# RajaeeKh/TriNerfLet

Measured on NVIDIA B200. Metric: rays/sec per training step (fwd+bwd), higher is better.
Workload: dtype f16

## Files before the change

### trinerflet_b200/csrc/idwt.cu

```cuda
#include "common.cuh"
#include "idwt_core.cuh"
#include <stdlib.h>

#include <type_traits>

namespace tnl {

template <typename Cfg, int W>
__global__ void __launch_bounds__(Cfg::NT, (768 / Cfg::NT) > 0 ? (768 / Cfg::NT) : 1)
k_idwt_fwd(const float* __restrict__ x, const float* __restrict__ yh, float* __restrict__ out, int n, int C,
           int rows_per_cta, float* __restrict__ abs_sum, const int4* __restrict__ items, const int* __restrict__ n_items) {
    extern __shared__ __align__(16) float smem[];
    float* mid0 = smem;
    float* stage0 = smem + 2 * Cfg::MID_F;
    const int tid = threadIdx.x;
    IdwtGeom g;
    if (items != nullptr) {
        const int chunks = C / Cfg::CG;
        const int idx = blockIdx.x / chunks;
        if (idx >= __ldg(n_items)) return;
        const int4 it = __ldg(items + idx);
        g = idwt_geom_item<Cfg>(tid, blockIdx.x % chunks, IdwtItem{it.x, it.y, it.z, it.w}, n, C);
    } else {
        g = idwt_geom<Cfg>(tid, IdwtBlock{(int)blockIdx.x, (int)blockIdx.y, (int)blockIdx.z}, n, C, rows_per_cta);
    }
    FwdState st;
    fwd_state_init<Cfg>(st, g, x, yh, tid);
    fwd_issue_stage<Cfg>(g, st, stage0, tid);
    fwd_issue_stage<Cfg>(g, st, stage0 + Cfg::STAGE, tid);
    for (int s = 0; s < g.nsteps; s += 3) {
#define TNL_STEP(PH)                                                                          \
    if (s + PH < g.nsteps) {                                                                  \
        const int ss = s + PH;                                                                \
        fwd_issue_stage<Cfg>(g, st, stage0 + ((PH + 2) % 3) * Cfg::STAGE, tid);               \
        cp_async_wait<2>();                                                                   \
        float* mid = mid0 + (ss & 1) * Cfg::MID_F;                                            \
        fwd_phase_a<Cfg, PH, W>(g, st, stage0 + PH * Cfg::STAGE, mid, tid, ss);               \
        __syncthreads();                                                                      \
        fwd_phase_b<Cfg, W>(g, st, mid, out, ss);                                             \
    }
        TNL_STEP(0) TNL_STEP(1) TNL_STEP(2)
#undef TNL_STEP
    }
    cp_async_wait<0>();
    if (abs_sum != nullptr) {
        float v = st.abs_acc;
#pragma unroll
        for (int o = 16; o > 0; o >>= 1) v += __shfl_xor_sync(0xffffffffu, v, o);
        __syncthreads();
        if ((tid & 31) == 0) smem[tid >> 5] = v;
        __syncthreads();
        if (tid < 32) {
            float w = tid < (Cfg::NT + 31) / 32 ? smem[tid] : 0.f;
#pragma unroll
            for (int o = 16; o > 0; o >>= 1) w += __shfl_xor_sync(0xffffffffu, w, o);
            if (tid == 0) atomicAdd(abs_sum, w);
        }
    }
}

template <typename Cfg, int W>
__global__ void __launch_bounds__(Cfg::NT, (768 / Cfg::NT) > 0 ? (768 / Cfg::NT) : 1)
k_idwt_bwd(const float* __restrict__ gout, float* __restrict__ g_x, float* __restrict__ g_yh, int n, int C,
           int rows_per_cta, const float* __restrict__ yh, const float* __restrict__ reg_grad, float reg_coef, int plane0,
           const int4* __restrict__ items, const int* __restrict__ n_items) {
    extern __shared__ __align__(16) float smem[];
    float* mid0 = smem;
    float* stage0 = smem + 2 * Cfg::MID_B;
    const int tid = threadIdx.x;
    IdwtGeom g;
    if (items != nullptr) {
        const int chunks = C / Cfg::CG;
        const int idx = blockIdx.x / chunks;
        if (idx >= __ldg(n_items)) return;
        const int4 it = __ldg(items + idx);
        g = idwt_geom_item<Cfg>(tid, blockIdx.x % chunks, IdwtItem{it.x, it.y, it.z, it.w}, n, C);
    } else {
        g = idwt_geom<Cfg>(tid, IdwtBlock{(int)blockIdx.x, (int)blockIdx.y, (int)blockIdx.z + plane0}, n, C, rows_per_cta);
    }
    BwdState st;
    bwd_state_init<Cfg>(st, g, gout);
    const float reg = (yh != nullptr && reg_grad != nullptr) ? reg_coef * __ldg(reg_grad) : 0.f;
    const float* yh_reg = (yh != nullptr && reg_grad != nullptr) ? yh : nullptr;
    bwd_issue_stage<Cfg>(g, st, stage0, tid);
    bwd_issue_stage<Cfg>(g, st, stage0 + Cfg::STAGE, tid);
    for (int s = 0; s < g.nsteps; s += 3) {
#define TNL_STEP(PH)                                                                          \
    if (s + PH < g.nsteps) {                                                                  \
        const int ss = s + PH;                                                                \
        bwd_issue_stage<Cfg>(g, st, stage0 + ((PH + 2) % 3) * Cfg::STAGE, tid);               \
        cp_async_wait<2>();                                                                   \
        float* mid = mid0 + (ss & 1) * Cfg::MID_B;                                            \
        bwd_phase_a<Cfg, PH, W>(st, stage0 + PH * Cfg::STAGE, mid, tid);                      \
        __syncthreads();                                                                      \
        bwd_phase_b<Cfg, W>(g, mid, g_x, g_yh, tid, ss, yh_reg, reg);                         \
    }
        TNL_STEP(0) TNL_STEP(1) TNL_STEP(2)
#undef TNL_STEP
    }
    cp_async_wait<0>();
}

__global__ void __launch_bounds__(256)
k_idwt_clean_fwd(const float* __restrict__ yh, int n, int C, const int4* __restrict__ items, const int* __restrict__ n_items,
                 float* __restrict__ abs_sum) {
    __shared__ float red[8];
    const int cnt = __ldg(n_items);
    const int warp = threadIdx.x >> 5, lane = threadIdx.x & 31;
    float acc = 0.f;
    const int run4 = 16 * C / 4;
    for (int idx = blockIdx.x; idx < cnt; idx += gridDim.x) {
        const int4 it = __ldg(items + idx);
        const int rows = min(it.w, n) - it.z;
        for (int rb = warp; rb < 3 * rows; rb += 8) {
            const int b = rb / rows, r = rb - b * rows;
            const float4* src = reinterpret_cast<const float4*>(yh + (((size_t)(it.x * 3 + b) * n + it.z + r) * n + it.y) * C);
            for (int q = lane; q < run4; q += 32) {
                const float4 v = __ldg(src + q);
                acc += fabsf(v.x) + fabsf(v.y) + fabsf(v.z) + fabsf(v.w);
            }
        }
    }
#pragma unroll
    for (int o = 16; o > 0; o >>= 1) acc += __shfl_xor_sync(0xffffffffu, acc, o);
    if (lane == 0) red[warp] = acc;
    __syncthreads();
    if (threadIdx.x < 32) {
        float w = threadIdx.x < 8 ? red[threadIdx.x] : 0.f;
// ... 74 lines not shown
    cudaFuncSetAttribute(k_idwt_bwd<Cfg, W>, cudaFuncAttributeMaxDynamicSharedMemorySize, (int)Cfg::SMEM_B);
    if (max_active > 0 && (parts & 1u))
        k_idwt_bwd<Cfg, W><<<max_active * (C / Cfg::CG), Cfg::NT, Cfg::SMEM_B, stream>>>(g, g_x, g_yh, (int)n, (int)C, 0, yh, reg_grad, reg_coef,
                                                                                     0, reinterpret_cast<const int4*>(active), counts);
    if (max_clean > 0 && (parts & 2u))
        k_idwt_clean_bwd<<<min(max_clean, (uint32_t)kNumSM * 8u), 256, 0, stream>>>(yh, g_x, g_yh, (int)n, (int)C,
                                                                                   reinterpret_cast<const int4*>(clean), counts + 1, reg_grad,
                                                                                   reg_coef, abs_sum);
    return finish_launch("idwt_level_backward_sparse");
}

template <typename Cfg, int W>
static int launch_fwd(const float* x, const float* yh, float* out, uint32_t n, uint32_t C, float* abs_sum,
                      cudaStream_t stream) {
    cudaFuncSetAttribute(k_idwt_fwd<Cfg, W>, cudaFuncAttributeMaxDynamicSharedMemorySize, (int)Cfg::SMEM_F);
    unsigned gx, gy, gz, rows;
    idwt_grid<Cfg>(n, C, kNumSM, gx, gy, gz, rows);
    k_idwt_fwd<Cfg, W><<<dim3(gx, gy, gz), Cfg::NT, Cfg::SMEM_F, stream>>>(x, yh, out, (int)n, (int)C, (int)rows, abs_sum, nullptr, nullptr);
    return finish_launch("idwt_level_forward");
}

template <typename Cfg, int W>
static int launch_bwd(const float* g, float* g_x, float* g_yh, uint32_t n, uint32_t C, const float* yh,
                      const float* reg_grad, float reg_coef, uint32_t plane0, uint32_t nplanes, cudaStream_t stream) {
    cudaFuncSetAttribute(k_idwt_bwd<Cfg, W>, cudaFuncAttributeMaxDynamicSharedMemorySize, (int)Cfg::SMEM_B);
    unsigned gx, gy, gz, rows;
    idwt_grid<Cfg>(n, C, kNumSM, gx, gy, gz, rows);
    gz = nplanes;
    k_idwt_bwd<Cfg, W><<<dim3(gx, gy, gz), Cfg::NT, Cfg::SMEM_B, stream>>>(g, g_x, g_yh, (int)n, (int)C, (int)rows, yh, reg_grad,
                                                                        reg_coef, (int)plane0, nullptr, nullptr);
    return finish_launch("idwt_level_backward");
}

template <typename Fn>
static int with_wavelet(uint32_t wavelet, Fn&& fn) {
    switch (wavelet) {
        case TNL_WAVELET_BIOR6_8: return fn(std::integral_constant<int, TNL_WAVELET_BIOR6_8>());
        case TNL_WAVELET_HAAR: return fn(std::integral_constant<int, TNL_WAVELET_HAAR>());
        case TNL_WAVELET_BIOR2_2: return fn(std::integral_constant<int, TNL_WAVELET_BIOR2_2>());
        case TNL_WAVELET_BIOR2_6: return fn(std::integral_constant<int, TNL_WAVELET_BIOR2_6>());
        case TNL_WAVELET_BIOR4_4: return fn(std::integral_constant<int, TNL_WAVELET_BIOR4_4>());
        default: set_error("idwt: unknown wavelet id %u", wavelet); return TNL_ERR_INVALID_ARGUMENT;
    }
}

}

using namespace tnl;

extern "C" {

int tnl_idwt_level_forward_wavelet(const float* x, const float* yh, float* out, uint32_t n, uint32_t C, float* abs_sum,
                                   uint32_t wavelet, tnl_stream_t stream) {
    TNL_ARG_CHECK(x && yh && out, "null pointer");
    TNL_ARG_CHECK(n >= 8 && n % 8 == 0 && n <= 16384, "n must be a multiple of 8 in [8, 16384]");
    TNL_ARG_CHECK(C >= 8 && C % 8 == 0, "C must be a multiple of 8");
    cudaStream_t s = reinterpret_cast<cudaStream_t>(stream);
    return with_wavelet(wavelet, [&](auto w) {
        constexpr int W = decltype(w)::value;
        if (C % 32 == 0 && getenv("TNL_IDWT_CG32")) return launch_fwd<IdwtCfg<32, 32>, W>(x, yh, out, n, C, abs_sum, s);
        if (C % 24 == 0) return launch_fwd<IdwtCfg<24, 32>, W>(x, yh, out, n, C, abs_sum, s);
        if (C % 16 == 0) return launch_fwd<IdwtCfg<16, 32>, W>(x, yh, out, n, C, abs_sum, s);
        return launch_fwd<IdwtCfg<8, 32>, W>(x, yh, out, n, C, abs_sum, s);
    });
}

int tnl_idwt_level_backward_wavelet(const float* g_out, float* g_x, float* g_yh, uint32_t n, uint32_t C, const float* yh,
                                    const float* reg_grad, float reg_coef, uint32_t plane0, uint32_t nplanes, uint32_t wavelet,
                                    tnl_stream_t stream) {
    TNL_ARG_CHECK(nplanes >= 1 && plane0 + nplanes <= 3, "plane range must lie in [0, 3)");
    TNL_ARG_CHECK(g_out && g_x && g_yh, "null pointer");
    TNL_ARG_CHECK(n >= 8 && n % 8 == 0 && n <= 16384, "n must be a multiple of 8 in [8, 16384]");
    TNL_ARG_CHECK(C >= 8 && C % 8 == 0, "C must be a multiple of 8");
    cudaStream_t s = reinterpret_cast<cudaStream_t>(stream);
    return with_wavelet(wavelet, [&](auto w) {
        constexpr int W = decltype(w)::value;
        if (C % 32 == 0 && getenv("TNL_IDWT_CG32"))
            return launch_bwd<IdwtCfg<32, 32>, W>(g_out, g_x, g_yh, n, C, yh, reg_grad, reg_coef, plane0, nplanes, s);
        if (C % 24 == 0) return launch_bwd<IdwtCfg<24, 32>, W>(g_out, g_x, g_yh, n, C, yh, reg_grad, reg_coef, plane0, nplanes, s);
        if (C % 16 == 0) return launch_bwd<IdwtCfg<16, 32>, W>(g_out, g_x, g_yh, n, C, yh, reg_grad, reg_coef, plane0, nplanes, s);
        return launch_bwd<IdwtCfg<8, 32>, W>(g_out, g_x, g_yh, n, C, yh, reg_grad, reg_coef, plane0, nplanes, s);
    });
}

int tnl_idwt_level_forward_sparse_wavelet(const float* x, const float* yh, float* out, uint32_t n, uint32_t C, float* abs_sum,
                                          const int32_t* active, const int32_t* clean, const int32_t* counts, uint32_t max_active,
                                          uint32_t max_clean, uint32_t parts, uint32_t wavelet, tnl_stream_t stream) {
    TNL_ARG_CHECK(x && yh && out && counts, "null pointer");
    TNL_ARG_CHECK(parts >= 1 && parts <= 3, "parts: bit 0 = active blocks, bit 1 = |yh| sum of the clean blocks");
    TNL_ARG_CHECK((max_active == 0 || active) && (max_clean == 0 || clean), "null work list");
    TNL_ARG_CHECK(n >= 16 && n % 16 == 0 && n <= 16384, "work-list mode: n must be a multiple of 16 in [16, 16384]");
    TNL_ARG_CHECK(C >= 8 && C % 8 == 0, "C must be a multiple of 8");
    cudaStream_t s = reinterpret_cast<cudaStream_t>(stream);
    return with_wavelet(wavelet, [&](auto w) {
        constexpr int W = decltype(w)::value;
        if (C % 24 == 0)
            return launch_fwd_sparse<IdwtCfg<24, 32>, W>(x, yh, out, n, C, abs_sum, active, clean, counts, max_active, max_clean, parts, s);
        if (C % 16 == 0)
            return launch_fwd_sparse<IdwtCfg<16, 32>, W>(x, yh, out, n, C, abs_sum, active, clean, counts, max_active, max_clean, parts, s);
        return launch_fwd_sparse<IdwtCfg<8, 32>, W>(x, yh, out, n, C, abs_sum, active, clean, counts, max_active, max_clean, parts, s);
    });
}

int tnl_idwt_level_backward_sparse_wavelet(const float* g_out, float* g_x, float* g_yh, uint32_t n, uint32_t C, const float* yh,
                                           const float* reg_grad, float reg_coef, const int32_t* active, const int32_t* clean,
                                           const int32_t* counts, uint32_t max_active, uint32_t max_clean, uint32_t parts,
                                           float* abs_sum, uint32_t wavelet, tnl_stream_t stream) {
    TNL_ARG_CHECK((g_out || !(parts & 1u)) && g_x && g_yh && counts, "null pointer");
    TNL_ARG_CHECK(parts >= 1 && parts <= 3, "parts: bit 0 = active blocks, bit 1 = clean blocks");
    TNL_ARG_CHECK((max_active == 0 || active) && (max_clean == 0 || clean), "null work list");
    TNL_ARG_CHECK(n >= 16 && n % 16 == 0 && n <= 16384, "work-list mode: n must be a multiple of 16 in [16, 16384]");
    TNL_ARG_CHECK(C >= 8 && C % 8 == 0, "C must be a multiple of 8");
    cudaStream_t s = reinterpret_cast<cudaStream_t>(stream);
    return with_wavelet(wavelet, [&](auto w) {
        constexpr int W = decltype(w)::value;
        if (C % 24 == 0)
            return launch_bwd_sparse<IdwtCfg<24, 32>, W>(g_out, g_x, g_yh, n, C, yh, reg_grad, reg_coef, active, clean, counts, max_active,
                                                         max_clean, parts, abs_sum, s);
        if (C % 16 == 0)
            return launch_bwd_sparse<IdwtCfg<16, 32>, W>(g_out, g_x, g_yh, n, C, yh, reg_grad, reg_coef, active, clean, counts, max_active,
                                                         max_clean, parts, abs_sum, s);
        return launch_bwd_sparse<IdwtCfg<8, 32>, W>(g_out, g_x, g_yh, n, C, yh, reg_grad, reg_coef, active, clean, counts, max_active,
                                                    max_clean, parts, abs_sum, s);
    });
}

int tnl_idwt_level_forward(const float* x, const float* yh, float* out, uint32_t n, uint32_t C, float* abs_sum,
                           tnl_stream_t stream) {
    return tnl_idwt_level_forward_wavelet(x, yh, out, n, C, abs_sum, TNL_WAVELET_BIOR6_8, stream);
}

int tnl_idwt_level_backward(const float* g_out, float* g_x, float* g_yh, uint32_t n, uint32_t C, const float* yh,
                            const float* reg_grad, float reg_coef, uint32_t plane0, uint32_t nplanes, tnl_stream_t stream) {
    return tnl_idwt_level_backward_wavelet(g_out, g_x, g_yh, n, C, yh, reg_grad, reg_coef, plane0, nplanes, TNL_WAVELET_BIOR6_8,
                                           stream);
}

int tnl_idwt_level_forward_sparse(const float* x, const float* yh, float* out, uint32_t n, uint32_t C, float* abs_sum,
                                  const int32_t* active, const int32_t* clean, const int32_t* counts, uint32_t max_active,
                                  uint32_t max_clean, uint32_t parts, tnl_stream_t stream) {
    return tnl_idwt_level_forward_sparse_wavelet(x, yh, out, n, C, abs_sum, active, clean, counts, max_active, max_clean, parts,
// ... 13 lines not shown
```

### trinerflet_b200/csrc/idwt_core.cuh

```cuda
#pragma once
#include <math.h>
#include <stddef.h>

#include "../../include/trinerflet_b200.h"

#ifdef __CUDACC__
#define TNL_HD __host__ __device__ __forceinline__
#else
#define TNL_HD inline
#endif

namespace tnl {

template <int W>
TNL_HD constexpr float rec_lo(int k);
template <int W>
TNL_HD constexpr float rec_hi(int k);

template <>
TNL_HD constexpr float rec_lo<TNL_WAVELET_BIOR6_8>(int k) {
    switch (k) {
        case 3: return 0.014426282505624435f;
        case 4: return 0.014467504896790148f;
        case 5: return -0.07872200106262882f;
// ... 113 lines not shown
TNL_HD constexpr float rec_hi<TNL_WAVELET_BIOR4_4>(int k) {
    switch (k) {
        case 5: return -0.03782845550726404f;
        case 6: return -0.023849465019556843f;
        case 7: return 0.11062440441843718f;
        case 8: return 0.37740285561283066f;
        case 9: return -0.8526986790088938f;
        case 10: return 0.37740285561283066f;
        case 11: return 0.11062440441843718f;
        case 12: return -0.023849465019556843f;
        case 13: return -0.03782845550726404f;
        default: return 0.0f;
    }
}

template <int W, bool HI>
TNL_HD constexpr bool wsyn_reaches(int i) {
    for (int e = 0; e < 2; ++e) {
        const int d = i - e;
        if (d < 0 || d > 8) continue;
        const float ge = HI ? rec_hi<W>(16 - 2 * d) : rec_lo<W>(16 - 2 * d);
        const float go = HI ? rec_hi<W>(17 - 2 * d) : rec_lo<W>(17 - 2 * d);
        if (ge != 0.f || go != 0.f) return true;
    }
    return false;
}

#if defined(__CUDA_ARCH__)
__device__ __forceinline__ void cp_async4(float* smem_dst, const float* gsrc, bool valid) {
    const unsigned d = (unsigned)__cvta_generic_to_shared(smem_dst);
    const int sz = valid ? 4 : 0;
    asm volatile("cp.async.ca.shared.global [%0], [%1], 4, %2;\n" ::"r"(d), "l"(gsrc), "r"(sz) : "memory");
}
__device__ __forceinline__ void cp_async_commit() { asm volatile("cp.async.commit_group;\n" ::: "memory"); }
template <int N>
__device__ __forceinline__ void cp_async_wait() { asm volatile("cp.async.wait_group %0;\n" ::"n"(N) : "memory"); }
#else
inline void cp_async4(float* smem_dst, const float* gsrc, bool valid) { *smem_dst = valid ? *gsrc : 0.0f; }
inline void cp_async_commit() {}
template <int N>
inline void cp_async_wait() {}
#endif

#if defined(__CUDA_ARCH__)
typedef float2 f2;
__device__ __forceinline__ f2 mk2(float a, float b) { return make_float2(a, b); }
__device__ __forceinline__ f2 fma2(float g, f2 w, f2 acc) { return __ffma2_rn(make_float2(g, g), w, acc); }
#else
struct f2 { float x, y; };
inline f2 mk2(float a, float b) { f2 r; r.x = a; r.y = b; return r; }
inline f2 fma2(float g, f2 w, f2 acc) { f2 r; r.x = fmaf(g, w.x, acc.x); r.y = fmaf(g, w.y, acc.y); return r; }
#endif

template <int CG_, int TW_>
struct IdwtCfg {
    static constexpr int CG = CG_;
    static constexpr int TW = TW_;
    static constexpr int TM = TW / 2;
    static constexpr int RA = 3;
    static constexpr int RB = 2 * RA;
    static constexpr int WIN = TM + 8;
    static constexpr int NT = WIN * CG;
    static constexpr int pad_to(int len) { return len + (((CG - len) % 32) + 32) % 32; }
    static constexpr int RS_F = pad_to(WIN * CG);
    static constexpr int RS_B = 2 * WIN * CG;
    static constexpr int MID_F = 2 * RB * RS_F;
    static constexpr int MID_B = 2 * RA * RS_B;
    static constexpr int STAGE = 4 * RA * NT;
    static constexpr int NSTAGE = 3;
    static constexpr size_t SMEM_F = sizeof(float) * (2 * MID_F + NSTAGE * STAGE);
    static constexpr size_t SMEM_B = sizeof(float) * (2 * MID_B + NSTAGE * STAGE);
    static_assert(CG % 2 == 0, "channel pairs");
    static_assert(RB * (TW / 4) * (CG / 2) == NT, "forward phase-B item count must equal the thread count");
    static_assert(RA * (TM / 2) * CG == NT, "backward phase-B item count must equal the thread count");
};

struct IdwtBlock {
    int bx, by, bz;
};

struct IdwtGeom {
    int n, C, plane, c0, m0, row_lo, row_hi, col, chan;
    int begin, end, nsteps;
};

template <typename Cfg>
TNL_HD IdwtGeom idwt_geom(int tid, IdwtBlock b, int n, int C, int rows_per_cta) {
    IdwtGeom g;
    g.n = n;
    g.C = C;
    const int chunks = C / Cfg::CG;
    g.plane = b.bz;
    g.c0 = (b.bx % chunks) * Cfg::CG;
    g.m0 = (b.bx / chunks) * Cfg::TM;
    g.row_lo = b.by * rows_per_cta;
    g.row_hi = g.row_lo + rows_per_cta < n ? g.row_lo + rows_per_cta : n;
    g.col = tid / Cfg::CG;
    g.chan = g.c0 + tid % Cfg::CG;
    g.begin = g.row_lo - 4;
    g.end = g.row_hi + 4;
    g.nsteps = (g.end - g.begin + Cfg::RA - 1) / Cfg::RA;
    return g;
}

struct IdwtItem {
    int plane, m0, row_lo, row_hi;
};

template <typename Cfg>
TNL_HD IdwtGeom idwt_geom_item(int tid, int chunk, IdwtItem it, int n, int C) {
    IdwtGeom g;
    g.n = n;
    g.C = C;
    g.plane = it.plane;
    g.c0 = chunk * Cfg::CG;
    g.m0 = it.m0;
    g.row_lo = it.row_lo;
    g.row_hi = it.row_hi < n ? it.row_hi : n;
    g.col = tid / Cfg::CG;
    g.chan = g.c0 + tid % Cfg::CG;
    g.begin = g.row_lo - 4;
    g.end = g.row_hi + 4;
    g.nsteps = (g.end - g.begin + Cfg::RA - 1) / Cfg::RA;
    return g;
}

struct FwdState {
    f2 wL[9];
    f2 wH[9];
    float abs_acc;
    const float *pLL, *pH0, *pH1, *pH2;
    int next_j;
    unsigned j_lim;
    bool col_ok;
    int b_lo, b_hi, b_r, b_sb;
    size_t b_out;
};

template <typename Cfg>
TNL_HD void fwd_state_init(FwdState& st, const IdwtGeom& g, const float* x, const float* yh, int tid) {
    for (int i = 0; i < 9; ++i) st.wL[i] = st.wH[i] = mk2(0.f, 0.f);
    st.abs_acc = 0.f;
    const int mcol = g.m0 - 4 + g.col;
    st.col_ok = mcol >= 0 && mcol < g.n;
    const long long plane_px = (long long)g.n * g.n;
    const long long row_stride = (long long)g.n * g.C;
    st.next_j = g.begin;
    st.j_lim = (unsigned)(g.end < g.n ? g.end : g.n);
    const long long off = (long long)(st.col_ok ? mcol : 0) * g.C + g.chan + (long long)g.begin * row_stride;
    st.pLL = x + (long long)g.plane * plane_px * g.C + off;
    st.pH0 = yh + (long long)(g.plane * 3 + 0) * plane_px * g.C + off;
    st.pH1 = yh + (long long)(g.plane * 3 + 1) * plane_px * g.C + off;
    st.pH2 = yh + (long long)(g.plane * 3 + 2) * plane_px * g.C + off;
    const int cp = tid % (Cfg::CG / 2), rs = tid / (Cfg::CG / 2);
    st.b_r = rs % Cfg::RB;
    st.b_sb = rs / Cfg::RB;
    st.b_lo = (0 * Cfg::RB + st.b_r) * Cfg::RS_F + (2 * st.b_sb) * Cfg::CG + 2 * cp;
// ... 10 lines not shown
    for (int rr = 0; rr < Cfg::RA; ++rr) {
        const bool ok = st.col_ok && (unsigned)(st.next_j + rr) < st.j_lim;
        cp_async4(d + rr * Cfg::NT * 4 + 0, st.pLL + rr * row_stride, ok);
        cp_async4(d + rr * Cfg::NT * 4 + 1, st.pH1 + rr * row_stride, ok);
        cp_async4(d + rr * Cfg::NT * 4 + 2, st.pH0 + rr * row_stride, ok);
        cp_async4(d + rr * Cfg::NT * 4 + 3, st.pH2 + rr * row_stride, ok);
    }
    cp_async_commit();
    st.next_j += Cfg::RA;
    st.pLL += Cfg::RA * row_stride;
    st.pH0 += Cfg::RA * row_stride;
    st.pH1 += Cfg::RA * row_stride;
    st.pH2 += Cfg::RA * row_stride;
}

template <int SLOT, int W = TNL_WAVELET_BIOR6_8>
TNL_HD void synth_rows(const f2 (&wL)[9], const f2 (&wH)[9], f2& even, f2& odd) {
    f2 e = mk2(0.f, 0.f), o = mk2(0.f, 0.f);
#pragma unroll
    for (int d = 0; d < 9; ++d) {
        const f2 l = wL[(SLOT + 1 + d) % 9], h = wH[(SLOT + 1 + d) % 9];
        const float ge0 = rec_lo<W>(16 - 2 * d), go0 = rec_lo<W>(17 - 2 * d);
        const float ge1 = rec_hi<W>(16 - 2 * d), go1 = rec_hi<W>(17 - 2 * d);
        if (ge0 != 0.f) e = fma2(ge0, l, e);
        if (go0 != 0.f) o = fma2(go0, l, o);
        if (ge1 != 0.f) e = fma2(ge1, h, e);
        if (go1 != 0.f) o = fma2(go1, h, o);
    }
    even = e;
    odd = o;
}

template <int SLOT, int W = TNL_WAVELET_BIOR6_8>
TNL_HD void fwd_row(FwdState& st, const float* stage, float* mid, int tid, int rr, int NT, int RB, int RS, bool own) {
    const f2* s = reinterpret_cast<const f2*>(stage + ((size_t)rr * NT + tid) * 4);
    f2 l = s[0];
    const f2 h = s[1];
    if (own) st.abs_acc += fabsf(l.y) + fabsf(h.x) + fabsf(h.y);
    l.x = l.x + l.x;
    st.wL[SLOT] = l;
    st.wH[SLOT] = h;
    f2 e, o;
    synth_rows<SLOT, W>(st.wL, st.wH, e, o);
    mid[(0 * RB + 2 * rr) * RS + tid] = e.x;
    mid[(0 * RB + 2 * rr + 1) * RS + tid] = o.x;
    mid[(1 * RB + 2 * rr) * RS + tid] = e.y;
    mid[(1 * RB + 2 * rr + 1) * RS + tid] = o.y;
}

template <typename Cfg, int PH, int W = TNL_WAVELET_BIOR6_8>
TNL_HD void fwd_phase_a(const IdwtGeom& g, FwdState& st, const float* stage, float* mid, int tid, int ss) {
    const bool col_own = g.col >= 4 && g.col < 4 + Cfg::TM;
    const int j0 = g.begin + ss * Cfg::RA;
    fwd_row<(PH * 3 + 0) % 9, W>(st, stage, mid, tid, 0, Cfg::NT, Cfg::RB, Cfg::RS_F, col_own && j0 + 0 >= g.row_lo && j0 + 0 < g.row_hi);
    fwd_row<(PH * 3 + 1) % 9, W>(st, stage, mid, tid, 1, Cfg::NT, Cfg::RB, Cfg::RS_F, col_own && j0 + 1 >= g.row_lo && j0 + 1 < g.row_hi);
    fwd_row<(PH * 3 + 2) % 9, W>(st, stage, mid, tid, 2, Cfg::NT, Cfg::RB, Cfg::RS_F, col_own && j0 + 2 >= g.row_lo && j0 + 2 < g.row_hi);
}

template <typename Cfg, int W = TNL_WAVELET_BIOR6_8>
TNL_HD void fwd_phase_b(const IdwtGeom& g, const FwdState& st, const float* mid, float* out, int ss) {
    const int r = st.b_r;
    const int m = g.begin + ss * Cfg::RA + (r >> 1) - 4;
    if (m < g.row_lo || m >= g.row_hi) return;
    const f2* mlo = reinterpret_cast<const f2*>(mid + st.b_lo);
    const f2* mhi = reinterpret_cast<const f2*>(mid + st.b_hi);
    f2 ev[2] = {mk2(0.f, 0.f), mk2(0.f, 0.f)}, od[2] = {mk2(0.f, 0.f), mk2(0.f, 0.f)};
#pragma unroll
    for (int i = 0; i < 10; ++i) {
        f2 h = mk2(0.f, 0.f), l = mk2(0.f, 0.f);
        if (wsyn_reaches<W, true>(i)) h = mhi[i * (Cfg::CG / 2)];
        if (wsyn_reaches<W, false>(i)) l = mlo[i * (Cfg::CG / 2)];
#pragma unroll
        for (int e = 0; e < 2; ++e) {
            const int d = i - e;
            if (d < 0 || d > 8) continue;
            const float ge0 = rec_lo<W>(16 - 2 * d), go0 = rec_lo<W>(17 - 2 * d);
            const float ge1 = rec_hi<W>(16 - 2 * d), go1 = rec_hi<W>(17 - 2 * d);
            if (ge0 != 0.f) ev[e] = fma2(ge0, l, ev[e]);
            if (go0 != 0.f) od[e] = fma2(go0, l, od[e]);
            if (ge1 != 0.f) ev[e] = fma2(ge1, h, ev[e]);
            if (go1 != 0.f) od[e] = fma2(go1, h, od[e]);
        }
    }
    const int Y = 2 * m + (r & 1);
    const int n2 = 2 * g.n;
    f2* orow = reinterpret_cast<f2*>(out + st.b_out + (size_t)Y * n2 * g.C);
#pragma unroll
    for (int e = 0; e < 2; ++e) {
        const int X = 2 * (g.m0 + 2 * st.b_sb + e);
// ... 27 lines not shown
    st.pb = gout + base + (long long)(st.okb ? Xb : 0) * g.C;
}

template <typename Cfg>
TNL_HD void bwd_issue_stage(const IdwtGeom& g, BwdState& st, float* stage, int tid) {
    const long long row_stride = (long long)(2 * g.n) * g.C;
    float* d = stage + (size_t)tid * 2;
#pragma unroll
    for (int rr = 0; rr < 2 * Cfg::RA; ++rr) {
        const bool rok = (unsigned)(st.next_y + rr) < st.y_lim;
        cp_async4(d + rr * Cfg::NT * 2 + 0, st.pa + rr * row_stride, rok && st.oka);
        cp_async4(d + rr * Cfg::NT * 2 + 1, st.pb + rr * row_stride, rok && st.okb);
    }
    cp_async_commit();
    st.next_y += 2 * Cfg::RA;
    st.pa += 2 * Cfg::RA * row_stride;
    st.pb += 2 * Cfg::RA * row_stride;
}

template <int SLOT, int W = TNL_WAVELET_BIOR6_8>
TNL_HD void analyse(const f2 (&w)[18], f2& a, f2& b) {
    f2 ra = mk2(0.f, 0.f), rb = mk2(0.f, 0.f);
#pragma unroll
    for (int k = 0; k < 18; ++k) {
        const f2 u = w[(SLOT + 1 + k) % 18];
        const float g0 = rec_lo<W>(k), g1 = rec_hi<W>(k);
        if (g0 != 0.f) ra = fma2(g0, u, ra);
        if (g1 != 0.f) rb = fma2(g1, u, rb);
    }
    a = ra;
    b = rb;
}

template <int SLOT, int W = TNL_WAVELET_BIOR6_8>
TNL_HD void bwd_row(BwdState& st, const float* stage, float* mid, int tid, int rr, int NT, int RS) {
    const f2* s = reinterpret_cast<const f2*>(stage);
    st.w[(SLOT + 17) % 18] = s[(size_t)(2 * rr) * NT + tid];
    st.w[SLOT] = s[(size_t)(2 * rr + 1) * NT + tid];
    f2 a, b;
    analyse<SLOT, W>(st.w, a, b);
    f2* m2 = reinterpret_cast<f2*>(mid);
    m2[(size_t)rr * RS + tid] = mk2(a.x, b.x);
    m2[(size_t)rr * RS + NT + tid] = mk2(a.y, b.y);
}

template <typename Cfg, int PH, int W = TNL_WAVELET_BIOR6_8>
TNL_HD void bwd_phase_a(BwdState& st, const float* stage, float* mid, int tid) {
    bwd_row<(2 * (PH * 3 + 0) + 1) % 18, W>(st, stage, mid, tid, 0, Cfg::NT, Cfg::RS_B);
    bwd_row<(2 * (PH * 3 + 1) + 1) % 18, W>(st, stage, mid, tid, 1, Cfg::NT, Cfg::RS_B);
    bwd_row<(2 * (PH * 3 + 2) + 1) % 18, W>(st, stage, mid, tid, 2, Cfg::NT, Cfg::RS_B);
}

TNL_HD float signf_(float v) { return v > 0.f ? 1.f : (v < 0.f ? -1.f : 0.f); }

template <typename Cfg, int W = TNL_WAVELET_BIOR6_8>
TNL_HD void bwd_phase_b(const IdwtGeom& g, const float* mid, float* g_x, float* g_yh, int tid, int ss, const float* yh,
                        float reg) {
    const int cb = tid % Cfg::CG;
    const int rs = tid / Cfg::CG;
    const int r = rs % Cfg::RA;
    const int sb = rs / Cfg::RA;
    const int m = g.begin + ss * Cfg::RA + r - 4;
    if (m < g.row_lo || m >= g.row_hi) return;
    const size_t plane_px = (size_t)g.n * g.n;
    const int w0 = g.m0 + 2 * sb;
    float y[2][3] = {{0.f, 0.f, 0.f}, {0.f, 0.f, 0.f}};
    if (yh != nullptr) {
#pragma unroll
        for (int e = 0; e < 2; ++e)
            if (w0 + e < g.n) {
                const size_t px = (size_t)m * g.n + w0 + e;
#pragma unroll
                for (int b = 0; b < 3; ++b) y[e][b] = yh[((size_t)(g.plane * 3 + b) * plane_px + px) * g.C + g.c0 + cb];
            }
    }
    const f2* mab = reinterpret_cast<const f2*>(mid) + (size_t)r * Cfg::RS_B + (4 * sb) * Cfg::CG + cb;
    f2 lo[2] = {mk2(0.f, 0.f), mk2(0.f, 0.f)}, hi[2] = {mk2(0.f, 0.f), mk2(0.f, 0.f)};
#pragma unroll
    for (int i = 0; i < 20; ++i) {
        const f2 v = mab[i * Cfg::CG];
#pragma unroll
        for (int e = 0; e < 2; ++e) {
            const int k = i - 2 * e;
            if (k < 0 || k > 17) continue;
            const float g0 = rec_lo<W>(k), g1 = rec_hi<W>(k);
            if (g0 != 0.f) lo[e] = fma2(g0, v, lo[e]);
            if (g1 != 0.f) hi[e] = fma2(g1, v, hi[e]);
        }
    }
#pragma unroll
    for (int e = 0; e < 2; ++e) {
        const int w = w0 + e;
        if (w < g.n) {
            const size_t px = (size_t)m * g.n + w;
            float lh = lo[e].y, hl = hi[e].x, hh = hi[e].y;
            if (yh != nullptr) {
                lh = fmaf(reg, signf_(y[e][0]), lh);
                hl = fmaf(reg, signf_(y[e][1]), hl);
                hh = fmaf(reg, signf_(y[e][2]), hh);
            }
            g_x[((size_t)g.plane * plane_px + px) * g.C + g.c0 + cb] = 2.0f * lo[e].x;
            g_yh[((size_t)(g.plane * 3 + 0) * plane_px + px) * g.C + g.c0 + cb] = lh;
            g_yh[((size_t)(g.plane * 3 + 1) * plane_px + px) * g.C + g.c0 + cb] = hl;
            g_yh[((size_t)(g.plane * 3 + 2) * plane_px + px) * g.C + g.c0 + cb] = hh;
        }
    }
}

template <typename Cfg>
inline void idwt_grid(unsigned n, unsigned C, unsigned num_sm, unsigned& gx, unsigned& gy, unsigned& gz, unsigned& rows) {
    gx = ((n + Cfg::TM - 1) / Cfg::TM) * (C / Cfg::CG);
    gz = 3;
    rows = 96;
    while (rows > 24 && gx * ((n + rows - 1) / rows) * gz < 4 * num_sm) rows /= 2;
    if (rows > n) rows = n;
    gy = (n + rows - 1) / rows;
}

}
```

Baseline: 11.93 million.

## Use 16-byte cp.async stages with deeper pipeline and prefetch yh in IDWT

Replaces the 4-byte cp.async staging in the dense IDWT forward and backward kernels with 16-byte cp.async.cg copies that use a transposed shared-memory layout and a configurable number of stages (NSTAGE). The wait now sits after phase A, so the next copy overlaps with compute. In backward, the regulariser's yh values for the next step are loaded early instead of inside phase B. The aim is fewer copy instructions and better latency hiding, at the cost of more shared memory per stage and a new requirement that inputs be 16-byte aligned. An A/B checking script is also added.

```diff
diff --git a/profiles/check_idwt_ab.py b/profiles/check_idwt_ab.py
--- /dev/null
+++ b/profiles/check_idwt_ab.py
@@ -0,0 +1,203 @@
+import argparse
+import ctypes
+import json
+import os
+import subprocess
+import sys
+
+sys.path.insert(0, os.path.dirname(os.path.dirname(os.path.abspath(__file__))))
+import torch
+
+from trinerflet_b200 import _lib, scene
+from trinerflet_b200.idwt_plan import WAVELET_IDS, IdwtPlan
+
+WAVES = ["bior6.8", "haar", "bior2.2", "bior2.6", "bior4.4"]
+N0, LEVELS, R, T = 64, 5, 2048, 64
+NAMES = ["tnl_idwt_level_forward_wavelet", "tnl_idwt_level_backward_wavelet", "tnl_idwt_level_forward_sparse_wavelet",
+         "tnl_idwt_level_backward_sparse_wavelet"]
+
+
+def open_lib(path):
+    lib = ctypes.CDLL(path)
+    for name in NAMES:
+        res, args = _lib.SIGNATURES[name]
+        getattr(lib, name).restype = res
+        getattr(lib, name).argtypes = args
+    return lib
+
+
+def card():
+    q = subprocess.run(["nvidia-smi", "--query-gpu=name,power.limit,clocks.max.sm", "--format=csv,noheader", "-i", "0"],
+                       capture_output=True, text=True).stdout.strip()
+    return dict(torch_name=torch.cuda.get_device_name(0), nvidia_smi=q)
+
+
+def P(t):
+    return None if t is None else ctypes.c_void_p(t.data_ptr())
+
+
+def run(lib, name, *args):
+    rc = getattr(lib, name)(*args, _lib.stream())
+    if rc != 0:
+        raise RuntimeError(f"{name}: rc={rc}")
+
+
+def fwd_dense(lib, w, x, yh, out, n, C, asum):
+    run(lib, NAMES[0], P(x), P(yh), P(out), n, C, P(asum), WAVELET_IDS[w])
+
+
+def bwd_dense(lib, w, g, gx, gyh, n, C, yh, rg):
+    run(lib, NAMES[1], P(g), P(gx), P(gyh), n, C, P(yh), P(rg), 0.25, 0, 3, WAVELET_IDS[w])
+
+
+def fwd_sparse(lib, w, s, x, yh, out, n, C, asum, parts):
+    run(lib, NAMES[2], P(x), P(yh), P(out), n, C, P(asum), P(s["active"]), P(s["clean"]), P(s["counts"]), s["cap_active"],
+        s["cap_clean"], parts, WAVELET_IDS[w])
+
+
+def bwd_sparse(lib, w, s, g, gx, gyh, n, C, yh, rg, asum, parts):
+    run(lib, NAMES[3], P(g), P(gx), P(gyh), n, C, P(yh), P(rg), 0.25, P(s["active"]), P(s["clean"]), P(s["counts"]),
+        s["cap_active"], s["cap_clean"], parts, P(asum), WAVELET_IDS[w])
+
+
+def make_plan(C):
+    bits = scene.packbits_cpu(scene.ball_density_grid(1.5, 0.75), 0.5).cuda()
+    flags = torch.empty(3 * T * T, dtype=torch.uint8, device="cuda")
+    _lib.call("tnl_mark_dirty_tiles", _lib.ptr(bits), 2, 128, 1.5, R, 32, 2, _lib.ptr(flags), _lib.stream())
+    return IdwtPlan(R, N0, LEVELS, C, "cuda").update(flags)
+
+
+def level_inputs(n, C, seed):
+    g = torch.Generator(device="cuda").manual_seed(seed)
+    x = torch.randn(3, n, n, C, device="cuda", generator=g)
+    yh = torch.randn(9, n, n, C, device="cuda", generator=g)
+    yh[yh.abs() < 0.05] = 0.0
+    gout = torch.randn(3, 2 * n, 2 * n, C, device="cuda", generator=g)
+    return x, yh, gout
+
+
+def check_identity(libs, report):
+    rg = torch.full((1,), 0.7, device="cuda")
+    worst = dict(max_abs_diff=0.0, abs_sum_rel=0.0, cases=0)
+    for C in (16, 32, 48):
+        plan = make_plan(C)
+        for w in WAVES:
+            for l in range(LEVELS):
+                n = N0 * 2 ** l
+                x, yh, gout = level_inputs(n, C, seed=1000 * C + 10 * l + WAVES.index(w))
+                res = []
+                for lib in libs:
+                    r = {}
+                    a = torch.zeros(4, device="cuda")
+                    r["out"] = torch.zeros(3, 2 * n, 2 * n, C, device="cuda")
+                    fwd_dense(lib, w, x, yh, r["out"], n, C, a[0:1])
+                    r["out_wl"] = torch.zeros_like(r["out"])
+                    fwd_sparse(lib, w, plan.fwd[l], x, yh, r["out_wl"], n, C, a[1:2], 3)
+                    for reg in (False, True):
+                        gx, gyh = torch.zeros(3, n, n, C, device="cuda"), torch.zeros(9, n, n, C, device="cuda")
+                        bwd_dense(lib, w, gout, gx, gyh, n, C, yh if reg else None, rg if reg else None)
+                        r[f"gx_{reg}"], r[f"gyh_{reg}"] = gx, gyh
+                        gx, gyh = torch.zeros_like(gx), torch.zeros_like(gyh)
+                        bwd_sparse(lib, w, plan.bwd[l], gout, gx, gyh, n, C, yh if reg else None, rg if reg else None,
+                                   a[2:3] if reg else None, 3)
+                        r[f"gx_wl_{reg}"], r[f"gyh_wl_{reg}"] = gx, gyh
+                    r["abs"] = a
+                    res.append(r)
+                torch.cuda.synchronize()
+                for k in res[0]:
+                    if k == "abs":
+                        rel = ((res[0][k] - res[1][k]).abs() / res[1][k].abs().clamp_min(1e-30)).max().item()
+                        worst["abs_sum_rel"] = max(worst["abs_sum_rel"], rel)
+                        if rel > 1e-6:
+                            raise SystemExit(f"|yh| sums differ: {w} C={C} level {l} rel {rel}")
+                        continue
+                    d = (res[0][k] - res[1][k]).abs().max().item()
+                    worst["max_abs_diff"] = max(worst["max_abs_diff"], d)
+                    if not torch.equal(res[0][k], res[1][k]):
+                        raise SystemExit(f"not bit-identical: {k} {w} C={C} level {l} max|d| {d}")
+                    worst["cases"] += 1
+                del res, x, yh, gout
+            print(f"identity C={C} {w}: ok", flush=True)
+    report["identity"] = worst
+
+
+def events_ms(fn, reps):
+    e0, e1 = torch.cuda.Event(enable_timing=True), torch.cuda.Event(enable_timing=True)
+    fn()
+    e0.record()
+    for _ in range(reps):
+        fn()
+    e1.record()
+    torch.cuda.synchronize()
+    return e0.elapsed_time(e1) / reps
+
+
+def timing(libs, labels, report, rounds, reps):
+    C, w = 32, "bior6.8"
+    plan = make_plan(C)
+    rg = torch.ones(1, device="cuda")
+    kinds = ["dense_fwd", "dense_bwd", "wl_fwd", "wl_bwd"]
+    best = {lab: {k: [float("inf")] * LEVELS for k in kinds} for lab in labels}
+    bytes_ = {k: [0] * LEVELS for k in kinds}
+    for l in range(LEVELS):
+        n = N0 * 2 ** l
+        x, yh, gout = level_inputs(n, C, seed=7 + l)
+        out = torch.empty(3, 2 * n, 2 * n, C, device="cuda")
+        gx, gyh = torch.empty(3, n, n, C, device="cuda"), torch.empty(9, n, n, C, device="cuda")
+        a = torch.zeros(1, device="cuda")
+        two_p = 2 * 3 * C * (2 * n) ** 2 * 4
+        bytes_["dense_fwd"][l] = bytes_["dense_bwd"][l] = two_p
+        fa, ba = plan.fwd[l], plan.bwd[l]
+        fns = {lab: dict(dense_fwd=lambda lib=lib: fwd_dense(lib, w, x, yh, out, n, C, a),
+                         dense_bwd=lambda lib=lib: bwd_dense(lib, w, gout, gx, gyh, n, C, yh, rg),
+                         wl_fwd=lambda lib=lib: fwd_sparse(lib, w, fa, x, yh, out, n, C, a, 1),
+                         wl_bwd=lambda lib=lib: bwd_sparse(lib, w, ba, gout, gx, gyh, n, C, yh, rg, None, 1))
+               for lab, lib in zip(labels, libs)}
+        for r in range(rounds):
+            for lab in (labels if r % 2 == 0 else labels[::-1]):
+                for k in kinds:
+                    best[lab][k][l] = min(best[lab][k][l], events_ms(fns[lab][k], reps))
+        del x, yh, gout, out, gx, gyh
+    res = {}
+    for lab in labels:
+        res[lab] = {}
+        for k in kinds:
+            t = best[lab][k]
+            row = dict(ms_per_level=[round(v, 4) for v in t], total_ms=round(sum(t), 4))
+            if k.startswith("dense"):
+                row["GBps_per_level"] = [round(b / v / 1e6, 1) for b, v in zip(bytes_[k], t)]
+            res[lab][k] = row
+        print(lab, {k: res[lab][k]["total_ms"] for k in kinds}, flush=True)
+        print(lab, "per level", {k: res[lab][k]["ms_per_level"] for k in kinds}, flush=True)
+    report["timing"] = dict(C=C, wavelet=w, rounds=rounds, reps=reps, method="CUDA events, min over rounds, libraries alternated",
+                            results=res)
+
+
+def main():
+    ap = argparse.ArgumentParser()
+    ap.add_argument("--other", required=True, help="the library to compare against (e.g. the parent commit's build)")
+    ap.add_argument("--out", default=None)
+    ap.add_argument("--rounds", type=int, default=5)
+    ap.add_argument("--reps", type=int, default=20)
+    ap.add_argument("--no-identity", action="store_true")
+    args = ap.parse_args()
+    if not torch.cuda.is_available():
+        raise SystemExit("check_idwt_ab: needs a CUDA device")
+    torch.backends.cuda.matmul.allow_tf32 = False
+    this = _lib.load()
+    other = open_lib(os.path.abspath(args.other))
+    libs, labels = [this, other], ["this", "other"]
+    report = dict(card=card(), this=_lib.LIB_PATH, other=os.path.abspath(args.other))
+    if not args.no_identity:
+        check_identity(libs, report)
+    timing(libs, labels, report, args.rounds, args.reps)
+    report["card_after"] = card()
+    if args.out:
+        os.makedirs(os.path.dirname(os.path.abspath(args.out)), exist_ok=True)
+        with open(args.out, "w") as f:
+            json.dump(report, f, indent=1)
+    print(json.dumps(dict(card=report["card"], identity=report.get("identity"))))
+
+
+if __name__ == "__main__":
+    main()
diff --git a/trinerflet_b200/csrc/idwt.cu b/trinerflet_b200/csrc/idwt.cu
--- a/trinerflet_b200/csrc/idwt.cu
+++ b/trinerflet_b200/csrc/idwt.cu
@@ -26,16 +26,20 @@
     }
     FwdState st;
     fwd_state_init<Cfg>(st, g, x, yh, tid);
-    fwd_issue_stage<Cfg>(g, st, stage0, tid);
-    fwd_issue_stage<Cfg>(g, st, stage0 + Cfg::STAGE, tid);
+    Stage16 cp = fwd_stage16_init<Cfg>(g, x, yh, tid);
+    const long long row_stride = (long long)n * C;
+#pragma unroll
+    for (int i = 0; i < Cfg::NSTAGE - 1; ++i) issue_stage16<Cfg, 1>(cp, stage0 + i * Cfg::STAGE, row_stride, tid);
+    cp_async_wait<Cfg::NSTAGE - 2>();
+    __syncthreads();
     for (int s = 0; s < g.nsteps; s += 3) {
 #define TNL_STEP(PH)                                                                          \
     if (s + PH < g.nsteps) {                                                                  \
         const int ss = s + PH;                                                                \
-        fwd_issue_stage<Cfg>(g, st, stage0 + ((PH + 2) % 3) * Cfg::STAGE, tid);               \
-        cp_async_wait<2>();                                                                   \
+        issue_stage16<Cfg, 1>(cp, stage0 + ((ss + Cfg::NSTAGE - 1) % Cfg::NSTAGE) * Cfg::STAGE, row_stride, tid); \
         float* mid = mid0 + (ss & 1) * Cfg::MID_F;                                            \
-        fwd_phase_a<Cfg, PH, W>(g, st, stage0 + PH * Cfg::STAGE, mid, tid, ss);               \
+        fwd_phase_a<Cfg, PH, W, true>(g, st, stage0 + (ss % Cfg::NSTAGE) * Cfg::STAGE, mid, tid, ss); \
+        cp_async_wait<Cfg::NSTAGE - 2>();                                                     \
         __syncthreads();                                                                      \
         fwd_phase_b<Cfg, W>(g, st, mid, out, ss);                                             \
     }
@@ -82,18 +86,25 @@
     bwd_state_init<Cfg>(st, g, gout);
     const float reg = (yh != nullptr && reg_grad != nullptr) ? reg_coef * __ldg(reg_grad) : 0.f;
     const float* yh_reg = (yh != nullptr && reg_grad != nullptr) ? yh : nullptr;
-    bwd_issue_stage<Cfg>(g, st, stage0, tid);
-    bwd_issue_stage<Cfg>(g, st, stage0 + Cfg::STAGE, tid);
+    Stage16 cp = bwd_stage16_init<Cfg>(g, gout, tid);
+    const long long row_stride = (long long)(2 * n) * C;
+#pragma unroll
+    for (int i = 0; i < Cfg::NSTAGE - 1; ++i) issue_stage16<Cfg, 2>(cp, stage0 + i * Cfg::STAGE, row_stride, tid);
+    float y[2][3] = {{0.f, 0.f, 0.f}, {0.f, 0.f, 0.f}};
+    bwd_reg_load<Cfg>(g, tid, 0, yh_reg, y);
+    cp_async_wait<Cfg::NSTAGE - 2>();
+    __syncthreads();
     for (int s = 0; s < g.nsteps; s += 3) {
 #define TNL_STEP(PH)                                                                          \
     if (s + PH < g.nsteps) {                                                                  \
         const int ss = s + PH;                                                                \
-        bwd_issue_stage<Cfg>(g, st, stage0 + ((PH + 2) % 3) * Cfg::STAGE, tid);               \
-        cp_async_wait<2>();                                                                   \
+        issue_stage16<Cfg, 2>(cp, stage0 + ((ss + Cfg::NSTAGE - 1) % Cfg::NSTAGE) * Cfg::STAGE, row_stride, tid); \
         float* mid = mid0 + (ss & 1) * Cfg::MID_B;                                            \
-        bwd_phase_a<Cfg, PH, W>(st, stage0 + PH * Cfg::STAGE, mid, tid);                      \
+        bwd_phase_a<Cfg, PH, W, true>(st, stage0 + (ss % Cfg::NSTAGE) * Cfg::STAGE, mid, tid); \
+        cp_async_wait<Cfg::NSTAGE - 2>();                                                     \
         __syncthreads();                                                                      \
-        bwd_phase_b<Cfg, W>(g, mid, g_x, g_yh, tid, ss, yh_reg, reg);                         \
+        bwd_phase_b_y<Cfg, W>(g, mid, g_x, g_yh, tid, ss, yh_reg, reg, y);                    \
+        bwd_reg_load<Cfg>(g, tid, ss + 1, yh_reg, y);                                         \
     }
         TNL_STEP(0) TNL_STEP(1) TNL_STEP(2)
 #undef TNL_STEP
@@ -234,6 +245,8 @@
     return finish_launch("idwt_level_backward");
 }
 
+static bool aligned16(const void* p) { return ((uintptr_t)p & 15u) == 0; }
+
 template <typename Fn>
 static int with_wavelet(uint32_t wavelet, Fn&& fn) {
     switch (wavelet) {
@@ -255,6 +268,7 @@
 int tnl_idwt_level_forward_wavelet(const float* x, const float* yh, float* out, uint32_t n, uint32_t C, float* abs_sum,
                                    uint32_t wavelet, tnl_stream_t stream) {
     TNL_ARG_CHECK(x && yh && out, "null pointer");
+    TNL_ARG_CHECK(aligned16(x) && aligned16(yh), "x and yh must be 16-byte aligned");
     TNL_ARG_CHECK(n >= 8 && n % 8 == 0 && n <= 16384, "n must be a multiple of 8 in [8, 16384]");
     TNL_ARG_CHECK(C >= 8 && C % 8 == 0, "C must be a multiple of 8");
     cudaStream_t s = reinterpret_cast<cudaStream_t>(stream);
@@ -272,6 +286,7 @@
                                     tnl_stream_t stream) {
     TNL_ARG_CHECK(nplanes >= 1 && plane0 + nplanes <= 3, "plane range must lie in [0, 3)");
     TNL_ARG_CHECK(g_out && g_x && g_yh, "null pointer");
+    TNL_ARG_CHECK(aligned16(g_out), "g_out must be 16-byte aligned");
     TNL_ARG_CHECK(n >= 8 && n % 8 == 0 && n <= 16384, "n must be a multiple of 8 in [8, 16384]");
     TNL_ARG_CHECK(C >= 8 && C % 8 == 0, "C must be a multiple of 8");
     cudaStream_t s = reinterpret_cast<cudaStream_t>(stream);
@@ -289,6 +304,7 @@
                                           const int32_t* active, const int32_t* clean, const int32_t* counts, uint32_t max_active,
                                           uint32_t max_clean, uint32_t parts, uint32_t wavelet, tnl_stream_t stream) {
     TNL_ARG_CHECK(x && yh && out && counts, "null pointer");
+    TNL_ARG_CHECK(aligned16(x) && aligned16(yh), "x and yh must be 16-byte aligned");
     TNL_ARG_CHECK(parts >= 1 && parts <= 3, "parts: bit 0 = active blocks, bit 1 = |yh| sum of the clean blocks");
     TNL_ARG_CHECK((max_active == 0 || active) && (max_clean == 0 || clean), "null work list");
     TNL_ARG_CHECK(n >= 16 && n % 16 == 0 && n <= 16384, "work-list mode: n must be a multiple of 16 in [16, 16384]");
@@ -309,6 +325,7 @@
                                            const int32_t* counts, uint32_t max_active, uint32_t max_clean, uint32_t parts,
                                            float* abs_sum, uint32_t wavelet, tnl_stream_t stream) {
     TNL_ARG_CHECK((g_out || !(parts & 1u)) && g_x && g_yh && counts, "null pointer");
+    TNL_ARG_CHECK(aligned16(g_out), "g_out must be 16-byte aligned");
     TNL_ARG_CHECK(parts >= 1 && parts <= 3, "parts: bit 0 = active blocks, bit 1 = clean blocks");
     TNL_ARG_CHECK((max_active == 0 || active) && (max_clean == 0 || clean), "null work list");
     TNL_ARG_CHECK(n >= 16 && n % 16 == 0 && n <= 16384, "work-list mode: n must be a multiple of 16 in [16, 16384]");
diff --git a/trinerflet_b200/csrc/idwt_core.cuh b/trinerflet_b200/csrc/idwt_core.cuh
--- a/trinerflet_b200/csrc/idwt_core.cuh
+++ b/trinerflet_b200/csrc/idwt_core.cuh
@@ -169,11 +169,19 @@
     const int sz = valid ? 4 : 0;
     asm volatile("cp.async.ca.shared.global [%0], [%1], 4, %2;\n" ::"r"(d), "l"(gsrc), "r"(sz) : "memory");
 }
+__device__ __forceinline__ void cp_async16(float* smem_dst, const float* gsrc, bool valid) {
+    const unsigned d = (unsigned)__cvta_generic_to_shared(smem_dst);
+    const int sz = valid ? 16 : 0;
+    asm volatile("cp.async.cg.shared.global [%0], [%1], 16, %2;\n" ::"r"(d), "l"(gsrc), "r"(sz) : "memory");
+}
 __device__ __forceinline__ void cp_async_commit() { asm volatile("cp.async.commit_group;\n" ::: "memory"); }
 template <int N>
 __device__ __forceinline__ void cp_async_wait() { asm volatile("cp.async.wait_group %0;\n" ::"n"(N) : "memory"); }
 #else
 inline void cp_async4(float* smem_dst, const float* gsrc, bool valid) { *smem_dst = valid ? *gsrc : 0.0f; }
+inline void cp_async16(float* smem_dst, const float* gsrc, bool valid) {
+    for (int i = 0; i < 4; ++i) smem_dst[i] = valid ? gsrc[i] : 0.0f;
+}
 inline void cp_async_commit() {}
 template <int N>
 inline void cp_async_wait() {}
@@ -204,7 +212,7 @@
     static constexpr int MID_F = 2 * RB * RS_F;
     static constexpr int MID_B = 2 * RA * RS_B;
     static constexpr int STAGE = 4 * RA * NT;
-    static constexpr int NSTAGE = 3;
+    static constexpr int NSTAGE = 4;
     static constexpr size_t SMEM_F = sizeof(float) * (2 * MID_F + NSTAGE * STAGE);
     static constexpr size_t SMEM_B = sizeof(float) * (2 * MID_B + NSTAGE * STAGE);
     static_assert(CG % 2 == 0, "channel pairs");
@@ -260,6 +268,56 @@
     g.end = g.row_hi + 4;
     g.nsteps = (g.end - g.begin + Cfg::RA - 1) / Cfg::RA;
     return g;
+}
+
+struct Stage16 {
+    const float* src;
+    int next;
+    unsigned lim;
+};
+
+template <typename Cfg>
+TNL_HD Stage16 fwd_stage16_init(const IdwtGeom& g, const float* x, const float* yh, int tid) {
+    constexpr int P = Cfg::CG / 4, RUN = Cfg::NT / 4;
+    const int b = tid / RUN, pix = (tid % RUN) / P, part = tid % P;
+    const int mcol = g.m0 - 4 + pix;
+    const bool col_ok = mcol >= 0 && mcol < g.n;
+    Stage16 s;
+    s.next = g.begin;
+    s.lim = col_ok ? (unsigned)(g.end < g.n ? g.end : g.n) : 0u;
+    const long long plane_px = (long long)g.n * g.n;
+    const long long off = (long long)(col_ok ? mcol : 0) * g.C + g.c0 + 4 * part + (long long)g.begin * g.n * g.C;
+    const float* base = b == 0 ? x + (long long)g.plane * plane_px * g.C
+                               : yh + (long long)(g.plane * 3 + (b == 1 ? 1 : b == 2 ? 0 : 2)) * plane_px * g.C;
+    s.src = base + off;
+    return s;
+}
+
+template <typename Cfg>
+TNL_HD Stage16 bwd_stage16_init(const IdwtGeom& g, const float* gout, int tid) {
+    constexpr int P = Cfg::CG / 4, ROW = Cfg::NT / 2;
+    const int h = tid / ROW, pix = (tid % ROW) / P, part = tid % P;
+    const int n2 = 2 * g.n;
+    const int X = 2 * g.m0 - 8 + pix;
+    const bool col_ok = X >= 0 && X < n2;
+    Stage16 s;
+    s.next = 2 * g.begin + h;
+    s.lim = col_ok ? (unsigned)(2 * g.end < n2 ? 2 * g.end : n2) : 0u;
+    const long long row_stride = (long long)n2 * g.C;
+    s.src = gout + (long long)g.plane * n2 * row_stride + (long long)s.next * row_stride + (long long)(col_ok ? X : 0) * g.C + g.c0 +
+            4 * part;
+    return s;
+}
+
+template <typename Cfg, int KROW>
+TNL_HD void issue_stage16(Stage16& s, float* stage, long long row_stride, int tid) {
+#pragma unroll
+    for (int k = 0; k < Cfg::RA; ++k)
+        cp_async16(stage + (size_t)k * 4 * Cfg::NT + 4 * tid, s.src + k * KROW * row_stride,
+                   (unsigned)(s.next + k * KROW) < s.lim);
+    cp_async_commit();
+    s.next += Cfg::RA * KROW;
+    s.src += Cfg::RA * KROW * row_stride;
 }
 
 struct FwdState {
@@ -336,10 +394,7 @@
 }
 
 template <int SLOT, int W = TNL_WAVELET_BIOR6_8>
-TNL_HD void fwd_row(FwdState& st, const float* stage, float* mid, int tid, int rr, int NT, int RB, int RS, bool own) {
-    const f2* s = reinterpret_cast<const f2*>(stage + ((size_t)rr * NT + tid) * 4);
-    f2 l = s[0];
-    const f2 h = s[1];
+TNL_HD void fwd_row_in(FwdState& st, f2 l, const f2 h, float* mid, int tid, int rr, int RB, int RS, bool own) {
     if (own) st.abs_acc += fabsf(l.y) + fabsf(h.x) + fabsf(h.y);
     l.x = l.x + l.x;
     st.wL[SLOT] = l;
@@ -352,13 +407,24 @@
     mid[(1 * RB + 2 * rr + 1) * RS + tid] = o.y;
 }
 
-template <typename Cfg, int PH, int W = TNL_WAVELET_BIOR6_8>
+template <int SLOT, int W = TNL_WAVELET_BIOR6_8, bool S16 = false>
+TNL_HD void fwd_row(FwdState& st, const float* stage, float* mid, int tid, int rr, int NT, int RB, int RS, bool own) {
+    if (S16) {
+        const float* s = stage + (size_t)rr * 4 * NT + tid;
+        fwd_row_in<SLOT, W>(st, mk2(s[0], s[NT]), mk2(s[2 * NT], s[3 * NT]), mid, tid, rr, RB, RS, own);
+    } else {
+        const f2* s = reinterpret_cast<const f2*>(stage + ((size_t)rr * NT + tid) * 4);
+        fwd_row_in<SLOT, W>(st, s[0], s[1], mid, tid, rr, RB, RS, own);
+    }
+}
+
+template <typename Cfg, int PH, int W = TNL_WAVELET_BIOR6_8, bool S16 = false>
 TNL_HD void fwd_phase_a(const IdwtGeom& g, FwdState& st, const float* stage, float* mid, int tid, int ss) {
     const bool col_own = g.col >= 4 && g.col < 4 + Cfg::TM;
     const int j0 = g.begin + ss * Cfg::RA;
-    fwd_row<(PH * 3 + 0) % 9, W>(st, stage, mid, tid, 0, Cfg::NT, Cfg::RB, Cfg::RS_F, col_own && j0 + 0 >= g.row_lo && j0 + 0 < g.row_hi);
-    fwd_row<(PH * 3 + 1) % 9, W>(st, stage, mid, tid, 1, Cfg::NT, Cfg::RB, Cfg::RS_F, col_own && j0 + 1 >= g.row_lo && j0 + 1 < g.row_hi);
-    fwd_row<(PH * 3 + 2) % 9, W>(st, stage, mid, tid, 2, Cfg::NT, Cfg::RB, Cfg::RS_F, col_own && j0 + 2 >= g.row_lo && j0 + 2 < g.row_hi);
+    fwd_row<(PH * 3 + 0) % 9, W, S16>(st, stage, mid, tid, 0, Cfg::NT, Cfg::RB, Cfg::RS_F, col_own && j0 + 0 >= g.row_lo && j0 + 0 < g.row_hi);
+    fwd_row<(PH * 3 + 1) % 9, W, S16>(st, stage, mid, tid, 1, Cfg::NT, Cfg::RB, Cfg::RS_F, col_own && j0 + 1 >= g.row_lo && j0 + 1 < g.row_hi);
+    fwd_row<(PH * 3 + 2) % 9, W, S16>(st, stage, mid, tid, 2, Cfg::NT, Cfg::RB, Cfg::RS_F, col_own && j0 + 2 >= g.row_lo && j0 + 2 < g.row_hi);
 }
 
 template <typename Cfg, int W = TNL_WAVELET_BIOR6_8>
@@ -452,11 +518,17 @@
     b = rb;
 }
 
-template <int SLOT, int W = TNL_WAVELET_BIOR6_8>
+template <int SLOT, int W = TNL_WAVELET_BIOR6_8, bool S16 = false>
 TNL_HD void bwd_row(BwdState& st, const float* stage, float* mid, int tid, int rr, int NT, int RS) {
-    const f2* s = reinterpret_cast<const f2*>(stage);
-    st.w[(SLOT + 17) % 18] = s[(size_t)(2 * rr) * NT + tid];
-    st.w[SLOT] = s[(size_t)(2 * rr + 1) * NT + tid];
+    if (S16) {
+        const float* s = stage + (size_t)rr * 4 * NT + tid;
+        st.w[(SLOT + 17) % 18] = mk2(s[0], s[NT]);
+        st.w[SLOT] = mk2(s[2 * NT], s[3 * NT]);
+    } else {
+        const f2* s = reinterpret_cast<const f2*>(stage);
+        st.w[(SLOT + 17) % 18] = s[(size_t)(2 * rr) * NT + tid];
+        st.w[SLOT] = s[(size_t)(2 * rr + 1) * NT + tid];
+    }
     f2 a, b;
     analyse<SLOT, W>(st.w, a, b);
     f2* m2 = reinterpret_cast<f2*>(mid);
@@ -464,18 +536,37 @@
     m2[(size_t)rr * RS + NT + tid] = mk2(a.y, b.y);
 }
 
-template <typename Cfg, int PH, int W = TNL_WAVELET_BIOR6_8>
+template <typename Cfg, int PH, int W = TNL_WAVELET_BIOR6_8, bool S16 = false>
 TNL_HD void bwd_phase_a(BwdState& st, const float* stage, float* mid, int tid) {
-    bwd_row<(2 * (PH * 3 + 0) + 1) % 18, W>(st, stage, mid, tid, 0, Cfg::NT, Cfg::RS_B);
-    bwd_row<(2 * (PH * 3 + 1) + 1) % 18, W>(st, stage, mid, tid, 1, Cfg::NT, Cfg::RS_B);
-    bwd_row<(2 * (PH * 3 + 2) + 1) % 18, W>(st, stage, mid, tid, 2, Cfg::NT, Cfg::RS_B);
+    bwd_row<(2 * (PH * 3 + 0) + 1) % 18, W, S16>(st, stage, mid, tid, 0, Cfg::NT, Cfg::RS_B);
+    bwd_row<(2 * (PH * 3 + 1) + 1) % 18, W, S16>(st, stage, mid, tid, 1, Cfg::NT, Cfg::RS_B);
+    bwd_row<(2 * (PH * 3 + 2) + 1) % 18, W, S16>(st, stage, mid, tid, 2, Cfg::NT, Cfg::RS_B);
 }
 
 TNL_HD float signf_(float v) { return v > 0.f ? 1.f : (v < 0.f ? -1.f : 0.f); }
 
+template <typename Cfg>
+TNL_HD void bwd_reg_load(const IdwtGeom& g, int tid, int ss, const float* yh, float (&y)[2][3]) {
+    const int cb = tid % Cfg::CG;
+    const int rs = tid / Cfg::CG;
+    const int r = rs % Cfg::RA;
+    const int sb = rs / Cfg::RA;
+    const int m = g.begin + ss * Cfg::RA + r - 4;
+    if (yh == nullptr || m < g.row_lo || m >= g.row_hi) return;
+    const size_t plane_px = (size_t)g.n * g.n;
+    const int w0 = g.m0 + 2 * sb;
+#pragma unroll
+    for (int e = 0; e < 2; ++e)
+        if (w0 + e < g.n) {
+            const size_t px = (size_t)m * g.n + w0 + e;
+#pragma unroll
+            for (int b = 0; b < 3; ++b) y[e][b] = yh[((size_t)(g.plane * 3 + b) * plane_px + px) * g.C + g.c0 + cb];
+        }
+}
+
 template <typename Cfg, int W = TNL_WAVELET_BIOR6_8>
-TNL_HD void bwd_phase_b(const IdwtGeom& g, const float* mid, float* g_x, float* g_yh, int tid, int ss, const float* yh,
-                        float reg) {
+TNL_HD void bwd_phase_b_y(const IdwtGeom& g, const float* mid, float* g_x, float* g_yh, int tid, int ss, const float* yh,
+                          float reg, const float (&y)[2][3]) {
     const int cb = tid % Cfg::CG;
     const int rs = tid / Cfg::CG;
     const int r = rs % Cfg::RA;
@@ -484,16 +575,6 @@
     if (m < g.row_lo || m >= g.row_hi) return;
     const size_t plane_px = (size_t)g.n * g.n;
     const int w0 = g.m0 + 2 * sb;
-    float y[2][3] = {{0.f, 0.f, 0.f}, {0.f, 0.f, 0.f}};
-    if (yh != nullptr) {
-#pragma unroll
-        for (int e = 0; e < 2; ++e)
-            if (w0 + e < g.n) {
-                const size_t px = (size_t)m * g.n + w0 + e;
-#pragma unroll
-                for (int b = 0; b < 3; ++b) y[e][b] = yh[((size_t)(g.plane * 3 + b) * plane_px + px) * g.C + g.c0 + cb];
-            }
-    }
     const f2* mab = reinterpret_cast<const f2*>(mid) + (size_t)r * Cfg::RS_B + (4 * sb) * Cfg::CG + cb;
     f2 lo[2] = {mk2(0.f, 0.f), mk2(0.f, 0.f)}, hi[2] = {mk2(0.f, 0.f), mk2(0.f, 0.f)};
 #pragma unroll
@@ -527,6 +608,14 @@
     }
 }
 
+template <typename Cfg, int W = TNL_WAVELET_BIOR6_8>
+TNL_HD void bwd_phase_b(const IdwtGeom& g, const float* mid, float* g_x, float* g_yh, int tid, int ss, const float* yh,
+                        float reg) {
+    float y[2][3] = {{0.f, 0.f, 0.f}, {0.f, 0.f, 0.f}};
+    bwd_reg_load<Cfg>(g, tid, ss, yh, y);
+    bwd_phase_b_y<Cfg, W>(g, mid, g_x, g_yh, tid, ss, yh, reg, y);
+}
+
 template <typename Cfg>
 inline void idwt_grid(unsigned n, unsigned C, unsigned num_sm, unsigned& gx, unsigned& gy, unsigned& gz, unsigned& rows) {
     gx = ((n + Cfg::TM - 1) / Cfg::TM) * (C / Cfg::CG);
```

New measurement: 11.97 million (median of 6 runs). About the same (+0.3%).
